# petim0/fly_bProject

Hardware: AMD Instinct MI355X
Metric: env-steps/sec (PPO rollout + update), 8192 envs per GPU (higher is better)
Workload: dtype f32 (optimizer step: fp16x2 operand split; rollout policy + critic: bf16x3 operand split; fp32 accumulate)

## Files before the change

fly_bproject_amd/_lib.py:

```python
import ctypes as C
import os

from .params import FlyParams

_HERE = os.path.dirname(os.path.abspath(__file__))
LIB_PATH = os.environ.get("FLYHIP_LIB") or os.path.join(_HERE, "libflyhip.so")
_lib = None


class FlyHipError(RuntimeError):
    pass


class FlyBuffers(C.Structure):
    _fields_ = [(n, C.c_void_p) for n in ("root", "dof_state", "targets", "contact", "pot", "prev_pot",
                                          "obs", "reward", "reset", "progress", "ep_return", "ep_length",
                                          "done_return", "done_length", "done_count")]


ABI_VERSION = 12
_P, _I, _L, _F = C.c_void_p, C.c_int, C.c_int64, C.c_float
SYMBOLS = {
    "fly_abi_version": [],
    "fly_create": [C.POINTER(FlyParams), C.POINTER(_P)],
# ... 11 lines not shown
    "ppo_step_bookkeeping": [_P, _L, _P, _F, _P, _I, _F, _F, _P],
    "ppo_rollout_step": [_P, _P, _P, _P, _P, _P, _P, _I, _F, _F, _P, _P, _P, _P, _P, _P],
    "ppo_rollout_all": [_P, _P, _P, _P, _P, _P, _P, _F, _F, _P, _P, _P, _P, _I, _P, _P, _P, _P, _P],
    "ppo_rollout_bookkeeping": [_P, _L, _L, _P, _P, _F, _P, _I, _F, _F, _P, _P],
    "mlp_forward": [_P, _P, _P, _L, _P, _P, _P, _P, _P, _P, _P, _P],
    "mlp_forward_sample": [_P, _P, _P, _L, _P, _P, _I, _F, _F, _P, _P, _P, _P, _P, _P],
    "mlp_grad_workspace_floats": [],
    "mlp_backward_dx": [_P] * 10 + [_L, _F, _F, _P, _P, _P, _P, _P, _P, _P],
    "mlp_forward_backward": [_P] * 4 + [_L] + [_P] * 9 + [_F, _F] + [_P] * 6 + [_I, _P, _P, _P, _I, _P],
    "mlp_grad_w": [_P] * 8 + [_L, _P, _P, _P, _P, _P, _P, _I, _P],
    "mlp_fused_workspace_floats": [],
    "mlp_fused_grad": [_P] * 3 + [_P, _L] + [_P] * 5 + [_F, _F] + [_P] * 6 + [C.POINTER(_P), _P],
    "mlp_fused_h2_workspace_floats": [],
    "mlp_fused_grad_h2": [_P] * 5 + [_I, _P, _L] + [_P] * 5 + [_F, _F] + [_P] * 6 + [C.POINTER(_P), _P],
    "mlp_h2_rescale": [_P] * 7,
    "mlp_adam_step": [_P] * 10 + [_F, _F, _F, _F, _F, _F, _P, _I, _P, _P, _P, _P, _P, _P] + [_P] * 3 + [_I, _P],
    "dqn_eps_greedy": [_P, _P, _P, _F, _I, _P, _L, _P],
    "dqn_huber_td": [_P, _P, _P, _P, _P, _F, _I, _L, _P, _P, _P],
    "dqn_forward": [_P, _P, _P, _L, _P, _P],
    "dqn_act": [_P, _P, _P, _L, _P, _P, _F, _P, _P, _P],
    "dqn_td_step": [_P] * 10 + [_L, _F, _F] + [_P] * 7,
    "dqn_grad_workspace_floats": [],
    "dqn_grad_w": [_P] * 6 + [_L, _P, _P, _I, _P],
    "dqn_fused_workspace_floats": [],
    "dqn_fused_image_halves": [_L],
    "dqn_fused_update": [_P] * 6 + [_I, _L, _F, _F, _P, _P, _P, _P, _I, _P],
    "dqn_fused_h2_workspace_floats": [],
    "dqn_fused_h2_image_halves": [_L],
    "dqn_fused_update_h2": [_P] * 10 + [_I, _L, _F, _F, _P, _P, _P, _P, _I, _I, _P],
    "dqn_adam_soft_update": [_P] * 12 + [_F, _F, _F, _F, _F, _P, _P, _P, _P, _P, _P, _P],
# ... 10 lines not shown
    import subprocess
    cmd = ["make", "-C", os.path.join(_HERE, "csrc"), "-j4"]
    if not verbose:
        cmd.insert(1, "-s")
    subprocess.check_call(cmd)


def load():
    global _lib
    if _lib is not None:
        return _lib
    if not os.path.exists(LIB_PATH):
        raise FlyHipError(
            "libflyhip.so is not built (%s). Run `python -c 'import __graft_entry__ as g; g.build()'` "
            "or `make -C fly_bproject_amd/csrc`. There is no CPU fallback." % LIB_PATH)
    lib = C.CDLL(LIB_PATH)
    lib.fly_last_error.restype = C.c_char_p
    lib.fly_last_error.argtypes = []
    for name, argtypes in SYMBOLS.items():
        fn = getattr(lib, name)
        fn.argtypes = argtypes
        fn.restype = C.c_int64 if name.endswith(("_workspace_floats", "_image_halves")) else C.c_int
    if lib.fly_abi_version() != ABI_VERSION:
        raise FlyHipError("stale libflyhip.so (ABI %d, this package was written for %d): rebuild it "
                          "(`make -C fly_bproject_amd/csrc`)" % (lib.fly_abi_version(), ABI_VERSION))
    _lib = lib
    return lib


def check(rc, what):
# ... 9 lines not shown
```

fly_bproject_amd/csrc/flyhip_abi.hip:

```cpp
#include <hip/hip_runtime.h>
#include <string.h>
#include <stdint.h>
#include <stdio.h>
#include <stdarg.h>
#include <new>
#include "flyhip.h"

extern "C" hipError_t flyhip_launch_env(int phases, const FlyConfig* dcfg, int n, const float* actions,
                                        const FlyBuffers* b, void* stream);
extern "C" hipError_t flyhip_launch_sample_logprob(const float* mu, const float* var, const float* eps,
                                                   float* act_out, float* logp_out, int64_t n, void* stream);
extern "C" hipError_t flyhip_launch_td_gae(const float* reward, const float* v, const float* v_next,
                                           const float* done, float gamma, float lambda, int64_t T, int64_t N,
                                           float* target_out, float* adv_out, int mode, void* stream);

extern "C" hipError_t flyhip_launch_mlp_forward(const float* P, const float* PF, const float* x, int64_t n, float* mu_out,
                                                float* v_out, float* out_save, float* h1_save, float* h2_save,
                                                float* h3_save, const uint16_t* PB, void* stream);

extern "C" hipError_t flyhip_launch_mlp_backward_dx(const float* PT, const float* out_saved, const float* h1,
                                                    const float* h2, const float* h3, const float* action,
                                                    const float* old_logp, const float* adv, const float* target,
                                                    const float* var, int64_t n, float inv_batch, float clip,
                                                    float* dz4, float* dz3, float* dz2, float* dz1, float* loss_part,
// ... 26 lines not shown
                                                   float* workspace, float* grad_out, const float* norm_mask, float* norm_ws,
                                                   int* norm_step, float* loss_part, float* const* dump, void* stream);
extern "C" hipError_t flyhip_launch_mlp_grad_w(const float* x, const float* h1, const float* h2, const float* h3,
                                               const float* dz1, const float* dz2, const float* dz3, const float* dz4,
                                               int64_t n, float* workspace, float* grad_out, const float* norm_mask,
                                               float* norm_ws, int* norm_step, const int* err, int gemm_b3, void* stream);
extern "C" hipError_t flyhip_launch_mlp_adam(float* P, float* PF, float* PT, const int* idx_f, const int* idx_t,
                                             const float* G, const float* mask, float* m,
                                             float* v, int* step, float lr, float beta1, float beta2, float eps,
                                             float max_norm, float grad_scale, float* norm_ws, int norm_ready,
                                             uint16_t* PB, uint16_t* PTB, const int* idx_fb, const int* idx_tb,
                                             int* step_out, const int* grad_invalid, uint16_t* PH, uint16_t* PTH,
                                             float* h2_scales, int h2_rescale, void* stream);
extern "C" hipError_t flyhip_launch_mlp_h2_rescale(const float* P, const int* idx_fb, const int* idx_tb, uint16_t* PH, uint16_t* PTH,
                                                   float* h2_scales, void* stream);
extern "C" int64_t flyhip_mlp_fused_h2_workspace_floats(void);
extern "C" hipError_t flyhip_launch_mlp_fused_grad_h2(const float* P, const uint16_t* PH, const uint16_t* PTH, float* fsc, int* ovf,
                                                      int freeze, const float* x, int64_t n, const float* action,
                                                      const float* old_logp, const float* adv, const float* target, const float* var,
                                                      float inv_batch, float clip, float* workspace, float* grad_out,
                                                      const float* norm_mask, float* norm_ws, int* norm_step, float* loss_part,
                                                      float* const* dump, void* stream);

extern "C" hipError_t flyhip_launch_bookkeeping(const float* reward, int64_t n, float* score_acc, float score_scale,
                                                float* action_var, int nvar, float var_decay, float var_min,
                                                void* stream);

extern "C" hipError_t flyhip_launch_dqn_eps_greedy(const float* q, const float* coin_u, const float* rand_u, float epsilon,
                                                   int A, float* act_out, int64_t n, void* stream);
extern "C" hipError_t flyhip_launch_dqn_huber_td(const float* q_table, const float* act, const float* reward,
// ... 376 lines not shown
    if (e != hipSuccess) return hip_fail(e, "mlp_fused_grad launch");
    return FLY_OK;
}

int64_t mlp_fused_h2_workspace_floats(void) { return flyhip_mlp_fused_h2_workspace_floats(); }

int mlp_h2_rescale(const float* params, const int32_t* idx_b3, const int32_t* idx_t_b3, uint16_t* params_h2, uint16_t* params_t_h2,
                   float* h2_scales, void* stream)
{
    if (!params || !idx_b3 || !idx_t_b3 || !params_h2 || !params_t_h2 || !h2_scales) return fail(FLY_E_ARG, "mlp_h2_rescale: null pointer");
    hipError_t e = flyhip_launch_mlp_h2_rescale(params, idx_b3, idx_t_b3, params_h2, params_t_h2, h2_scales, stream);
    if (e != hipSuccess) return hip_fail(e, "mlp_h2_rescale launch");
    return FLY_OK;
}

int mlp_fused_grad_h2(const float* params, const uint16_t* params_h2, const uint16_t* params_t_h2, float* h2_scales,
                      int32_t* h2_overflow, int32_t freeze, const float* x, int64_t n, const float* action,
                      const float* old_logp, const float* adv, const float* target, const float* var, float inv_batch,
                      float clip, float* workspace, float* grad, const float* norm_mask, float* norm_ws, int32_t* norm_step,
                      float* loss_part, float* const* debug_dump, void* stream)
{
    if ((norm_ws != nullptr) != (norm_mask != nullptr) || (norm_ws != nullptr) != (norm_step != nullptr))
        return fail(FLY_E_ARG, "mlp_fused_grad_h2: norm_mask, norm_ws and norm_step go together");
    if (!params || !params_h2 || !params_t_h2 || !h2_scales || !h2_overflow)
        return fail(FLY_E_ARG, "mlp_fused_grad_h2: needs params, both fp16x2 plane buffers, the scale table and the overflow word");
    if (!x || !action || !old_logp || !adv || !target || !var || !workspace || !grad)
        return fail(FLY_E_ARG, "mlp_fused_grad_h2: null pointer");
    if (n <= 0) return fail(FLY_E_ARG, "mlp_fused_grad_h2: n must be > 0");
    if (debug_dump) {
        if (!debug_dump[0]) return fail(FLY_E_ARG, "mlp_fused_grad_h2: debug_dump[0] is null");
// ... 6 lines not shown
                                                   loss_part, debug_dump, stream);
    if (e != hipSuccess) return hip_fail(e, "mlp_fused_grad_h2 launch");
    return FLY_OK;
}

int mlp_adam_step(float* params, float* params_frag, float* params_t_frag, const int32_t* idx_frag,
                  const int32_t* idx_t_frag, const float* grad, const float* mask, float* exp_avg,
                  float* exp_avg_sq, int32_t* step, float lr, float beta1, float beta2, float eps,
                  float max_norm, float grad_scale, float* norm_ws, int32_t norm_ready, uint16_t* params_b3,
                  uint16_t* params_t_b3, const int32_t* idx_b3, const int32_t* idx_t_b3, int32_t* step_out,
                  const int32_t* grad_invalid, uint16_t* params_h2, uint16_t* params_t_h2, float* h2_scales, int32_t h2_rescale,
                  void* stream)
{
    if (params_b3 && (!params_t_b3 || !idx_b3 || !idx_t_b3))
        return fail(FLY_E_ARG, "mlp_adam_step: params_b3 needs params_t_b3, idx_b3 and idx_t_b3");
    if (params_h2 && (!params_t_h2 || !h2_scales || !params_b3))
        return fail(FLY_E_ARG, "mlp_adam_step: params_h2 needs params_t_h2, h2_scales and the bf16x3 planes with their index maps");
    if (!params || !params_frag || !params_t_frag || !idx_frag || !idx_t_frag || !grad || !mask || !exp_avg ||
        !exp_avg_sq || !step || !norm_ws)
        return fail(FLY_E_ARG, "mlp_adam_step: null pointer");
    hipError_t e = flyhip_launch_mlp_adam(params, params_frag, params_t_frag, idx_frag, idx_t_frag, grad, mask, exp_avg, exp_avg_sq, step, lr, beta1, beta2,
                                          eps, max_norm, grad_scale, norm_ws, norm_ready, params_b3, params_t_b3, idx_b3, idx_t_b3,
                                          step_out, grad_invalid, params_h2, params_t_h2, h2_scales, h2_rescale, stream);
    if (e != hipSuccess) return hip_fail(e, "mlp_adam_step launch");
    return FLY_OK;
}

int dqn_eps_greedy(const float* q, const float* coin_u, const float* rand_u, float epsilon, int32_t A,
                   float* act_out, int64_t n, void* stream)
{
    if (!q || !coin_u || !rand_u || !act_out) return fail(FLY_E_ARG, "dqn_eps_greedy: null pointer");
    if (n <= 0 || A < 2) return fail(FLY_E_ARG, "dqn_eps_greedy: need n > 0 and A >= 2");
    hipError_t e = flyhip_launch_dqn_eps_greedy(q, coin_u, rand_u, epsilon, A, act_out, n, stream);
// ... 199 lines not shown
```

fly_bproject_amd/csrc/mlp_adam.inc:

```
#ifndef ADAM_THREADS_AB
#define ADAM_THREADS_AB 1024
#endif
constexpr int ADAM_THREADS = ADAM_THREADS_AB;
constexpr int ADAM_WAVES = ADAM_THREADS / 64;
constexpr int ADAM_BLOCKS = (MLP_PACKED_FLOATS + ADAM_THREADS - 1) / ADAM_THREADS;

__global__ __launch_bounds__(ADAM_THREADS) void mlp_adam_norm_kernel(const float* __restrict__ G,
                                                                     const float* __restrict__ mask, float grad_scale,
                                                                     float* __restrict__ norm_ws, int* __restrict__ step,
                                                                     const int* __restrict__ grad_invalid)
{
    __shared__ float red[ADAM_WAVES];
    if (G[MLP_ERR_SLOT] != 0.0f) return;
    if (grad_invalid && *grad_invalid != 0) return;
    const int tid = threadIdx.x;
    const int i = blockIdx.x * ADAM_THREADS + tid;
    float ss = 0.0f;
    if (i < MLP_PACKED_FLOATS) { const float g = G[i] * grad_scale * mask[i]; ss = g * g; }
    for (int o = 32; o > 0; o >>= 1) ss += __shfl_down(ss, o, 64);
    if ((tid & 63) == 0) red[tid >> 6] = ss;
    __syncthreads();
    if (tid == 0) {
        float t = 0.0f;
        for (int w = 0; w < ADAM_WAVES; ++w) t += red[w];
// ... 12 lines not shown
                                                                      const int* __restrict__ step, float lr, float beta1,
                                                                      float beta2, float eps, float max_norm,
                                                                      float grad_scale, float* __restrict__ norm_ws,
                                                                      int nparts, float part_scale,
                                                                      u16* __restrict__ PB, u16* __restrict__ PTB,
                                                                      const int* __restrict__ idx_fb,
                                                                      const int* __restrict__ idx_tb,
                                                                      int* __restrict__ step_out,
                                                                      const int* __restrict__ grad_invalid,
                                                                      u16* __restrict__ PH, u16* __restrict__ PTH,
                                                                      float* __restrict__ fsc, int h2_rescale)
{
    __shared__ float s_coef, s_step_size, s_bc2_sqrt;
    __shared__ float red[ADAM_WAVES];
    __shared__ float s_wscale[4];
    __shared__ unsigned s_wmax[4];
    const int tid = threadIdx.x;
    const bool self_norm = step_out != nullptr;
    if (G[MLP_ERR_SLOT] != 0.0f || (grad_invalid && *grad_invalid != 0)) {
        if (self_norm && blockIdx.x == 0 && tid == 0) *step_out = *step;
        return;
    }
    const int i = blockIdx.x * ADAM_THREADS + tid;
    const bool live = i < MLP_PACKED_FLOATS;
    const float mk = live ? mask[i] : 0.0f, g_in = live ? G[i] : 0.0f, m_in = live ? m[i] : 0.0f, v_in = live ? v[i] : 0.0f,
                p_in = live ? P[i] : 0.0f;
    const int jf = live ? idx_f[i] : -1, jt = live ? idx_t[i] : -1;
    {
        float t = 0.0f;
        if (self_norm) {
            const float4* g4 = reinterpret_cast<const float4*>(G);
            const float4* m4 = reinterpret_cast<const float4*>(mask);
            for (int q = tid; q < MLP_PACKED_FLOATS / 4; q += ADAM_THREADS) {
                const float4 g = g4[q], k = m4[q];
                const float a = g.x * grad_scale * k.x, b = g.y * grad_scale * k.y, c = g.z * grad_scale * k.z, d = g.w * grad_scale * k.w;
                t += (a * a + b * b) + (c * c + d * d);
            }
        } else
        for (int b = tid; b < nparts; b += ADAM_THREADS) t += norm_ws[1 + b];
        for (int o = 32; o > 0; o >>= 1) t += __shfl_down(t, o, 64);
        if ((tid & 63) == 0) red[tid >> 6] = t;
    }
    if (PH && !h2_rescale && tid < 4) s_wscale[tid] = fsc[8 + tid];
    if (PH && h2_rescale) {
        if (tid < 4) s_wmax[tid] = 0u;
        __syncthreads();
        float mx[4] = {0.0f, 0.0f, 0.0f, 0.0f};
        const float4* p4 = reinterpret_cast<const float4*>(P);
        for (int q = tid; q < MLP_PACKED_FLOATS / 4; q += ADAM_THREADS) {
            const int o = 4 * q;
            const int l = o < MLP_OFF_B1 ? 0 : o < MLP_OFF_W2 ? -1 : o < MLP_OFF_B2 ? 1 : o < MLP_OFF_W3 ? -1 : o < MLP_OFF_B3 ? 2 : o < MLP_OFF_W4 ? -1
                        : o < MLP_OFF_B4 ? 3 : -1;
            const float4 w = p4[q];
            const float a = fmaxf(fmaxf(fabsf(w.x), fabsf(w.y)), fmaxf(fabsf(w.z), fabsf(w.w)));
#pragma unroll
            for (int k = 0; k < 4; ++k) mx[k] = l == k ? fmaxf(mx[k], a) : mx[k];
        }
#pragma unroll
        for (int k = 0; k < 4; ++k) {
            float m = mx[k];
#pragma unroll
            for (int o = 32; o > 0; o >>= 1) m = fmaxf(m, __shfl_xor(m, o, 64));
            if ((tid & 63) == 0 && m > 0.0f) atomicMax(&s_wmax[k], __float_as_uint(m));
        }
        __syncthreads();
        if (tid < 4) {
            const float m = fminf(fmaxf(__uint_as_float(s_wmax[tid]), 0x1p-4f), 0x1p60f);
            const float sc = ldexpf(1.0f, 11 - ilogbf(m));
            s_wscale[tid] = sc;
            if (blockIdx.x == 0) { fsc[8 + tid] = sc; fsc[16 + 8 + tid] = 1.0f / sc; }
        }
    }
    __syncthreads();
    if (tid == 0) {
        float t = 0.0f;
        for (int w = 0; w < ADAM_WAVES; ++w) t += red[w];
        t *= part_scale;
        const float norm = sqrtf(t);
        const float coef = max_norm / (norm + 1e-6f);
        s_coef = coef < 1.0f ? coef : 1.0f;
        if (blockIdx.x == 0) norm_ws[0] = norm;
        const int step_now = self_norm ? *step + 1 : *step;
        if (self_norm && blockIdx.x == 0) *step_out = step_now;
        const float ts = (float)step_now;
        const float bc1 = 1.0f - powf(beta1, ts);
        const float bc2 = 1.0f - powf(beta2, ts);
// ... 2 lines not shown
    }
    __syncthreads();
    if (!live) return;
    const float coef = s_coef * grad_scale;
    const float step_size = s_step_size;
    const float bc2_sqrt = s_bc2_sqrt;
    const float g = g_in * coef * mk;
    const float mi = beta1 * m_in + (1.0f - beta1) * g;
    const float vi = beta2 * v_in + (1.0f - beta2) * g * g;
    m[i] = mi; v[i] = vi;
    const float denom = sqrtf(vi) / bc2_sqrt + eps;
    const float p = p_in - mk * (step_size * (mi / denom));
    P[i] = p;
    if (jf >= 0) PF[jf] = p;
    if (jt >= 0) PT[jt] = p;
    int kf = -1, kt = -1;
    if (PB) {
        u16 a, b, c;
        split3(p, a, b, c);
        kf = idx_fb[i]; kt = idx_tb[i];
        if (kf >= 0) { PB[kf] = a; PB[kf + 512] = b; PB[kf + 1024] = c; }
        if (kt >= 0) { PTB[kt] = a; PTB[kt + 512] = b; PTB[kt + 1024] = c; }
    }
    if (PH && kf >= 0) {
        const int layer = i < MLP_OFF_W2 ? 0 : i < MLP_OFF_W3 ? 1 : i < MLP_OFF_W4 ? 2 : 3;
        const float ps = p * s_wscale[layer];
        const _Float16 h0 = (_Float16)ps;
        const _Float16 h1 = (_Float16)(ps - (float)h0);
        const u16 a = __builtin_bit_cast(u16, h0), b = __builtin_bit_cast(u16, h1);
        const int hf = (kf / 1536) * 1024 + kf % 1536;
        PH[hf] = a; PH[hf + 512] = b;
        if (kt >= 0) { const int ht = (kt / 1536) * 1024 + kt % 1536; PTH[ht] = a; PTH[ht + 512] = b; }
    }
}

constexpr int H2_RESCALE_THREADS = 1024;
__global__ __launch_bounds__(H2_RESCALE_THREADS) void mlp_h2_rescale_kernel(const float* __restrict__ P, const int* __restrict__ idx_fb,
                                                                            const int* __restrict__ idx_tb, u16* __restrict__ PH,
                                                                            u16* __restrict__ PTH, float* __restrict__ fsc)
{
    __shared__ unsigned s_max[4];
    __shared__ float s_scale[4];
    const int tid = threadIdx.x;
    if (tid < 4) s_max[tid] = 0u;
    __syncthreads();
    float mine[4] = {0.0f, 0.0f, 0.0f, 0.0f};
    for (int i = tid; i < MLP_PACKED_FLOATS; i += H2_RESCALE_THREADS)
        if (idx_fb[i] >= 0) {
// ... 36 lines not shown
```

fly_bproject_amd/csrc/mlp_mfma.hip:

```cpp
#include <hip/hip_runtime.h>
#include <stdint.h>
#include <type_traits>
#include <cstdio>
#include <cstdlib>
#include "flyhip.h"
#include "mlp_layout.h"

namespace {

#include "mlp_gemm.inc"
#include "fs_stamp.inc"
#include "mlp_forward.inc"
#include "mlp_backward.inc"
#include "mlp_grad_w.inc"
#include "mlp_fused_step.inc"
#include "mlp_adam.inc"
#include "fly_body.inc"

constexpr int RS_LDS_FLOATS = FWD_LDS_FLOATS > ENVS_PER_BLOCK * FLY_NUM_OBS ? FWD_LDS_FLOATS : ENVS_PER_BLOCK * FLY_NUM_OBS;
constexpr int RS_B3_LDS_FLOATS = FWD_B3_LDS_FLOATS > ENVS_PER_BLOCK * FLY_NUM_OBS ? FWD_B3_LDS_FLOATS : ENVS_PER_BLOCK * FLY_NUM_OBS;
static_assert(ENVS_PER_BLOCK == BM && BLOCK == THREADS, "one forward tile = one env block");

template <bool B3>
__global__ __launch_bounds__(THREADS, B3 ? 1 : 2) void rollout_step_kernel(
// ... 450 lines not shown
                                             float* h2_scales, int h2_rescale, void* stream)
{
    int nparts = ADAM_BLOCKS;
    float part_scale = 1.0f;
    if (step_out) {
        part_scale = 1.0f;
    } else if (norm_ready) {
        nparts = RED_BLOCKS;
        part_scale = grad_scale * grad_scale;
    } else {
        hipLaunchKernelGGL(mlp_adam_norm_kernel, dim3(ADAM_BLOCKS), dim3(ADAM_THREADS), 0, (hipStream_t)stream, G, mask,
                           grad_scale, norm_ws, step, grad_invalid);
        hipError_t e = hipGetLastError();
        if (e != hipSuccess) return e;
    }
    hipLaunchKernelGGL(mlp_adam_apply_kernel, dim3(ADAM_BLOCKS), dim3(ADAM_THREADS), 0, (hipStream_t)stream, P, PF, PT,
                       idx_f, idx_t, G, mask, m, v, step, lr, beta1, beta2, eps, max_norm, grad_scale, norm_ws, nparts,
                       part_scale, PB, PTB, idx_fb, idx_tb, step_out, grad_invalid, PH, PTH, h2_scales, h2_rescale);
    return hipGetLastError();
}

extern "C" hipError_t flyhip_launch_mlp_h2_rescale(const float* P, const int* idx_fb, const int* idx_tb, uint16_t* PH, uint16_t* PTH,
                                                   float* h2_scales, void* stream)
{
    hipLaunchKernelGGL(mlp_h2_rescale_kernel, dim3(1), dim3(H2_RESCALE_THREADS), 0, (hipStream_t)stream, P, idx_fb, idx_tb, PH, PTH, h2_scales);
    return hipGetLastError();
}
```

fly_bproject_amd/policy.py:

```python
import ctypes as C
import os

import torch

from . import _lib

IN, IN_PAD, H1, H2, H3, OUT, NACT = 73, 80, 256, 128, 128, 32, 18
OFF_W1 = 0
OFF_B1 = OFF_W1 + H1 * IN_PAD
OFF_W2 = OFF_B1 + H1
OFF_B2 = OFF_W2 + H2 * H1
OFF_W3 = OFF_B2 + H2
OFF_B3 = OFF_W3 + H3 * H2
OFF_W4 = OFF_B3 + H3
OFF_B4 = OFF_W4 + OUT * H3
PACKED = OFF_B4 + OUT
ERR_SLOT = OFF_W1 + 76
OFF_F1 = 0
OFF_F2 = OFF_F1 + H1 * IN_PAD
OFF_F3 = OFF_F2 + H2 * H1
OFF_F4 = OFF_F3 + H3 * H2
FRAG = OFF_F4 + OUT * H3
OFF_TF2 = 0
OFF_TF3 = OFF_TF2 + H1 * H2
# ... 50 lines not shown
        src = off_w + n * K + k
        if li == 1:
            idx_fb[src] = OFF_PB[li] + (k // 128) * (3 * N * 128) + _plane_index(n, k % 128, 128)
        else:
            idx_fb[src] = OFF_PB[li] + _plane_index(n, k, K)
        if OFF_PTB[li] is not None:
            idx_tb[src] = OFF_PTB[li] + _plane_index(k, n, N)
    for idx, size in ((idx_fb, PB_HALVES), (idx_tb, PTB_HALVES)):
        used = idx[idx >= 0].astype(np.int64)
        allpos = np.concatenate([used, used + 512, used + 1024])
        assert len(np.unique(allpos)) == len(allpos) and allpos.max() < size
    assert 3 * (idx_fb >= 0).sum() == PB_HALVES and 3 * (idx_tb >= 0).sum() == PTB_HALVES
    return idx_fb, idx_tb


PH_HALVES, PTH_HALVES = PB_HALVES * 2 // 3, PTB_HALVES * 2 // 3
H2_SCALE_FLOATS, H2_INV, H2_W0 = 48, 16, 8
H2_CLASSES = ("x", "h1", "h2", "h3", "dz4", "dz3", "dz2", "dz1")


def split_f16x2(w, scale):
    y = w * scale
    h0 = y.to(torch.float16)
    h1 = (y - h0.float()).to(torch.float16)
    return [t.view(torch.int16) for t in (h0, h1)]


def h2_weight_scale(wmax):
    import math
    m = min(max(float(wmax), 2.0 ** -4), 2.0 ** 60)
# ... 9 lines not shown


def split_bf16x3(w):
    w0 = w.to(torch.bfloat16)
    r1 = w - w0.float()
    w1 = r1.to(torch.bfloat16)
    w2 = (r1 - w1.float()).to(torch.bfloat16)
    return [t.view(torch.int16) for t in (w0, w1, w2)]


class PackedPolicy:
    def __init__(self, net, device):
        self.device = torch.device(device)
        self._lib = _lib.load()
        self.P = torch.zeros(PACKED, dtype=torch.float32, device=self.device)
        self.PF = torch.zeros(FRAG, dtype=torch.float32, device=self.device)
        self.PT = torch.zeros(FRAG_T, dtype=torch.float32, device=self.device)
        env_gemm = os.environ.get("FLY_GEMM")
        self._gemm = "bf16x3" if env_gemm in (None, "f16x2") else env_gemm
        self.gemm_infer = os.environ.get("FLY_GEMM_INFER", self._gemm)
        assert self._gemm in ("f32", "bf16x3") and self.gemm_infer in ("f32", "bf16x3")
        self.PB = torch.zeros(PB_HALVES, dtype=torch.int16, device=self.device)
        self.PTB = torch.zeros(PTB_HALVES, dtype=torch.int16, device=self.device)
        self._step_gemm = os.environ.get("FLY_STEP_GEMM", "f16x2" if env_gemm in (None, "f16x2") else "bf16x3")
        assert self._step_gemm in ("bf16x3", "f16x2")
        self.PH = torch.zeros(PH_HALVES, dtype=torch.int16, device=self.device)
        self.PTH = torch.zeros(PTH_HALVES, dtype=torch.int16, device=self.device)
        self.h2_scales = torch.zeros(H2_SCALE_FLOATS, dtype=torch.float32, device=self.device)
        self.h2_overflow = torch.zeros(1, dtype=torch.int32, device=self.device)
        self.h2_freeze = False
        self.h2_calibrated = False
        self._h2_steps_since_rescale = 0
        self.h2_suspended = False
        self.h2_overflows = 0
        self._h2_reset_scales()
        idx_fb, idx_tb = build_plane_maps()
        self.idx_fb = torch.from_numpy(idx_fb).to(self.device)
        self.idx_tb = torch.from_numpy(idx_tb).to(self.device)
        self._src_fb = torch.nonzero(self.idx_fb >= 0).squeeze(-1)
        self._dst_fb = self.idx_fb[self._src_fb].long()
        self._src_tb = torch.nonzero(self.idx_tb >= 0).squeeze(-1)
        self._dst_tb = self.idx_tb[self._src_tb].long()
        idx_f, idx_t = build_index_maps()
        self.idx_f = torch.from_numpy(idx_f).to(self.device)
        self.idx_t = torch.from_numpy(idx_t).to(self.device)
        self._src_f = torch.nonzero(self.idx_f >= 0).squeeze(-1)
        self._dst_f = self.idx_f[self._src_f].long()
        self._src_t = torch.nonzero(self.idx_t >= 0).squeeze(-1)
        self._dst_t = self.idx_t[self._src_t].long()
        P = self.P
        self.W1 = P[OFF_W1:OFF_B1].view(H1, IN_PAD)
        self.b1 = P[OFF_B1:OFF_W2]
        self.W2 = P[OFF_W2:OFF_B2].view(H2, H1)
        self.b2 = P[OFF_B2:OFF_W3]
        self.W3 = P[OFF_W3:OFF_B3].view(H3, H2)
        self.b3 = P[OFF_B3:OFF_W4]
        self.W4 = P[OFF_W4:OFF_B4].view(OUT, H3)
        self.b4 = P[OFF_B4:PACKED]
        self.views = {
            "shared_net.0.weight": self.W1[:, :IN], "shared_net.0.bias": self.b1,
            "shared_net.2.weight": self.W2, "shared_net.2.bias": self.b2,
            "to_mean.0.weight": self.W3[:64], "to_mean.0.bias": self.b3[:64],
            "to_value.0.weight": self.W3[64:], "to_value.0.bias": self.b3[64:],
            "to_mean.2.weight": self.W4[:NACT, :64], "to_mean.2.bias": self.b4[:NACT],
# ... 2 lines not shown
        params = dict(net.named_parameters())
        assert set(params) == set(self.views), "Net does not have the reference's parameter set"
        with torch.no_grad():
            for k, view in self.views.items():
                view.copy_(params[k].data.to(self.device))
                params[k].data = view
        mask = torch.zeros(PACKED, dtype=torch.float32, device=self.device)
        for k, view in self.views.items():
            off = view.storage_offset()
            idx = torch.arange(PACKED, device=self.device).as_strided(view.shape, view.stride(), off)
            mask[idx.reshape(-1)] = 1.0
        self.grad_mask = mask
        assert int(mask.sum().item()) == 69587
        self.refresh()

    def refresh(self):
        with torch.no_grad():
            self.PF[self._dst_f] = self.P[self._src_f]
            self.PT[self._dst_t] = self.P[self._src_t]
            self._refresh_planes()
        self.version += 1

    refresh_transposes = refresh

    def _refresh_planes(self):
        with torch.no_grad():
            for dst_buf, src, dst in ((self.PB, self._src_fb, self._dst_fb), (self.PTB, self._src_tb, self._dst_tb)):
                for term, plane in enumerate(split_bf16x3(self.P[src])):
                    dst_buf[dst + 512 * term] = plane

        if self.h2_live():
# ... 6 lines not shown
        s = torch.ones(H2_SCALE_FLOATS)
        s[:4] = 2.0 ** 4
        s[4:8] = 2.0 ** 28
        s[H2_INV:H2_INV + 16] = 1.0 / s[:16]
        s[32:] = 0.0
        self.h2_scales.copy_(s)
        self.h2_calibrated = False

    def _refresh_planes_h2(self):
        if self.device.type != "cuda":
            return
        p = lambda t: C.c_void_p(t.data_ptr())
        _lib.check(self._lib.mlp_h2_rescale(p(self.P), p(self.idx_fb), p(self.idx_tb), p(self.PH), p(self.PTH), p(self.h2_scales),
                                            _lib.stream_ptr()), "mlp_h2_rescale")
        self._h2_steps_since_rescale = 0

    def _planes_live(self):
        return self._gemm == "bf16x3" or self.gemm_infer == "bf16x3"

    @property
    def step_gemm(self):
        return self._step_gemm if self._gemm == "bf16x3" else self._gemm

    @step_gemm.setter
    def step_gemm(self, mode):
        assert mode in ("bf16x3", "f16x2")
        was = self.h2_live()
        self._step_gemm = mode
        if self.h2_live() and not was:
            self._refresh_planes_h2()
# ... 18 lines not shown
        elif self.h2_live() and not was_h2:
            self._refresh_planes_h2()
    version = 0

    def _plane_args(self):
        if not self._planes_live():
            return (None, None, None, None)
        p = lambda t: C.c_void_p(t.data_ptr())
        return (p(self.PB), p(self.PTB), p(self.idx_fb), p(self.idx_tb))

    def _h2_args(self):
        if not self.h2_live():
            return (None, None, None, C.c_int(0))
        p = lambda t: C.c_void_p(t.data_ptr())
        rescale = self._h2_steps_since_rescale >= max(1, min(64, int(0.9 / (3.2 * self.lr))))
        self._h2_steps_since_rescale = 1 if rescale else self._h2_steps_since_rescale + 1
        return (p(self.PH), p(self.PTH), p(self.h2_scales), C.c_int(1 if rescale else 0))

    def pb_ptr(self):
        return C.c_void_p(self.PB.data_ptr()) if self.gemm == "bf16x3" else None

    def infer_pb_ptr(self):
        return C.c_void_p(self.PB.data_ptr()) if self.gemm_infer == "bf16x3" else None

    def ptb_ptr(self):
        return C.c_void_p(self.PTB.data_ptr()) if self.gemm == "bf16x3" else None

    def forward(self, x, want_mu=True, want_v=True, saves=None):
        lead = x.shape[:-1]
        x2 = x.reshape(-1, IN)
# ... 155 lines not shown
        return (parts[0] + parts[1]) / n

    @property
    def step(self):
        return self._step2[self._step_idx:self._step_idx + 1]

    def adam_step(self, grad_scale=1.0, norm_ready=False, self_norm=False, grad_invalid=None):
        p = lambda t: C.c_void_p(t.data_ptr())
        self.version += 1
        self.steps_issued += 1
        step_in = self.step
        step_out = None
        if self_norm:
            self._step_idx ^= 1
            step_out = p(self.step)
        _lib.check(self._lib.mlp_adam_step(p(self.P), p(self.PF), p(self.PT), p(self.idx_f), p(self.idx_t), p(self.G),
                                           p(self.grad_mask), p(self.exp_avg),
                                           p(self.exp_avg_sq), p(step_in), C.c_float(self.lr),
                                           C.c_float(self.betas[0]), C.c_float(self.betas[1]), C.c_float(self.eps),
                                           C.c_float(self.max_norm), C.c_float(grad_scale), p(self._norm_ws),
                                           C.c_int(1 if norm_ready else 0), *self._plane_args(), step_out,
                                           p(grad_invalid) if grad_invalid is not None else None, *self._h2_args(), _lib.stream_ptr()),
                   "mlp_adam_step")
```

fly_bproject_amd/ppo.py:

```python
import ctypes as C
import collections
import os

import torch
import torch.nn as nn
import torch.nn.functional as F

from . import _lib
from .fly import Fly
from .params import NUM_DOF


class Net(nn.Module):

    def __init__(self, num_obs, num_act):
        super().__init__()
        self.shared_net = nn.Sequential(nn.Linear(num_obs, 256), nn.ELU(), nn.Linear(256, 128), nn.ELU())
        self.to_mean = nn.Sequential(nn.Linear(128, 64), nn.ELU(), nn.Linear(64, num_act), nn.ELU())
        self.to_value = nn.Sequential(nn.Linear(128, 64), nn.ELU(), nn.Linear(64, 1))

    _policy = None

    def pi(self, x):
        if self._policy is not None and not torch.is_grad_enabled():
# ... 279 lines not shown
                pol.check_fused_launch()
            if short == 0:
                break
            if short < 0 or short > len(slices) or attempt == 2:
                raise _lib.FlyHipError("update: device step counter is %d steps behind the %d issued" % (short, pol.steps_issued))
            pol.steps_issued -= short
            if h2 and not pol.h2_suspended:
                pol.h2_overflow.zero_()
                pol.h2_suspended = True
                pol.h2_calibrated = False
                pol.h2_overflows += 1
            else:
                pol.fuse_fwd_bwd = False
                print("mlp_forward_backward: %d of %d optimizer steps were refused on the device (a backward workgroup "
                      "could not get its tile); redoing them with two launches" % (short, len(slices)))
            run(slices[len(slices) - short:])
            if self._p2p is not None and not self._p2p.check():
                raise _lib.FlyHipError("dp_allreduce_p2p: a rank never published its gradient while refused steps were redone")
        pol.h2_suspended = False
        self.optim_step += len(slices)
        self._drain_log(block=True)
        self._finish_update(sync_grads)

    def _finish_update(self, sync_grads):
        import torch.distributed as dist
        pol = self.policy
        if self.world_size > 1 and not sync_grads:
            for buf in (pol.P, pol.exp_avg, pol.exp_avg_sq):
                dist.all_reduce(buf, op=dist.ReduceOp.SUM)
                buf.div_(self.world_size)
            pol.refresh()

    def prepare(self):
        if getattr(self, "_prepared", False):
            return
        self._prepared = True
        self.p2p_selftest = None
        sync_grads = self.world_size > 1 and self.dp_mode == "grad_allreduce"
        if sync_grads and self.update_backend == "hip" and self.dp_allreduce in ("p2p", "auto"):
            self._p2p = self._open_p2p(self.policy.G.numel())

# ... 257 lines not shown
```

include/flyhip.h:

```cpp
#ifndef FLYHIP_H
#define FLYHIP_H

#include <stdint.h>

#ifdef __cplusplus
extern "C" {
#endif

#define FLY_NUM_DOF 18
#define FLY_NUM_OBS 73
#define FLY_NUM_LEGS 6
#define FLY_NUM_ABDOMEN 5
#define FLY_NUM_CONTACT 11
#define FLY_ROOT_DIM 13

#define FLY_OK 0
#define FLY_E_ARG (-1)
#define FLY_E_HIP (-2)
#define FLY_E_CONFIG (-3)

#define PPO_GAE_COMPAT 0
#define PPO_GAE_DONE_PER_STEP 1
#define PPO_GAE_MASK_RECURRENCE 2
#define PPO_GAE_SCAN 4
// ... 134 lines not shown
                   float inv_batch, float clip, float* workspace, float* grad, const float* norm_mask, float* norm_ws,
                   int32_t* norm_step, float* loss_part, float* const* debug_dump, void* stream);
int mlp_adam_step(float* params, float* params_frag, float* params_t_frag, const int32_t* idx_frag,
                  const int32_t* idx_t_frag, const float* grad, const float* mask, float* exp_avg,
                  float* exp_avg_sq, int32_t* step, float lr, float beta1, float beta2, float eps,
                  float max_norm, float grad_scale, float* norm_ws, int32_t norm_ready,
                  uint16_t* params_b3, uint16_t* params_t_b3, const int32_t* idx_b3,
                  const int32_t* idx_t_b3, int32_t* step_out, const int32_t* grad_invalid,
                  uint16_t* params_h2, uint16_t* params_t_h2, float* h2_scales, int32_t h2_rescale, void* stream);

#define MLP_PH_HALVES_ABI 147456
#define MLP_PTH_HALVES_ABI 106496
#define MLP_H2_SCALE_FLOATS_ABI 48
int mlp_h2_rescale(const float* params, const int32_t* idx_b3, const int32_t* idx_t_b3, uint16_t* params_h2, uint16_t* params_t_h2,
                   float* h2_scales, void* stream);
int64_t mlp_fused_h2_workspace_floats(void);
int mlp_fused_grad_h2(const float* params, const uint16_t* params_h2, const uint16_t* params_t_h2, float* h2_scales,
                      int32_t* h2_overflow, int32_t freeze, const float* x, int64_t n, const float* action,
                      const float* old_logp, const float* adv, const float* target, const float* var, float inv_batch,
                      float clip, float* workspace, float* grad, const float* norm_mask, float* norm_ws, int32_t* norm_step,
                      float* loss_part, float* const* debug_dump, void* stream);


int dqn_eps_greedy(const float* q, const float* coin_u, const float* rand_u, float epsilon, int32_t A,
                   float* act_out, int64_t n, void* stream);
int dqn_huber_td(const float* q_table, const float* act, const float* reward, const float* q_next,
                 const float* done, float discount, int32_t A, int64_t B, float* dq, float* loss_part,
                 void* stream);

#define DQN_QB_HALVES_ABI 282624
// ... 51 lines not shown
```

Before: 68.06 million.

## Defer fp32/bf16x3 plane writes out of Adam into a lazy refresh kernel

```diff
diff --git a/fly_bproject_amd/_lib.py b/fly_bproject_amd/_lib.py
--- a/fly_bproject_amd/_lib.py
+++ b/fly_bproject_amd/_lib.py
@@ -49,6 +49,7 @@
     "mlp_fused_h2_workspace_floats": [],
     "mlp_fused_grad_h2": [_P] * 5 + [_I, _P, _L] + [_P] * 5 + [_F, _F] + [_P] * 6 + [C.POINTER(_P), _P],
     "mlp_h2_rescale": [_P] * 7,
+    "mlp_plane_refresh": [_P] * 7,
     "mlp_adam_step": [_P] * 10 + [_F, _F, _F, _F, _F, _F, _P, _I, _P, _P, _P, _P, _P, _P] + [_P] * 3 + [_I, _P],
     "dqn_eps_greedy": [_P, _P, _P, _F, _I, _P, _L, _P],
     "dqn_huber_td": [_P, _P, _P, _P, _P, _F, _I, _L, _P, _P, _P],
@@ -89,6 +90,7 @@
         raise FlyHipError(
             "libflyhip.so is not built (%s). Run `python -c 'import __graft_entry__ as g; g.build()'` "
             "or `make -C fly_bproject_amd/csrc`. There is no CPU fallback." % LIB_PATH)
+    import torch
     lib = C.CDLL(LIB_PATH)
     lib.fly_last_error.restype = C.c_char_p
     lib.fly_last_error.argtypes = []
diff --git a/fly_bproject_amd/csrc/flyhip_abi.hip b/fly_bproject_amd/csrc/flyhip_abi.hip
--- a/fly_bproject_amd/csrc/flyhip_abi.hip
+++ b/fly_bproject_amd/csrc/flyhip_abi.hip
@@ -64,6 +64,8 @@
                                              float* h2_scales, int h2_rescale, void* stream);
 extern "C" hipError_t flyhip_launch_mlp_h2_rescale(const float* P, const int* idx_fb, const int* idx_tb, uint16_t* PH, uint16_t* PTH,
                                                    float* h2_scales, void* stream);
+extern "C" hipError_t flyhip_launch_mlp_plane_refresh(const float* P, const int* src, float* PF, float* PT, uint16_t* PB, uint16_t* PTB,
+                                                     void* stream);
 extern "C" int64_t flyhip_mlp_fused_h2_workspace_floats(void);
 extern "C" hipError_t flyhip_launch_mlp_fused_grad_h2(const float* P, const uint16_t* PH, const uint16_t* PTH, float* fsc, int* ovf,
                                                       int freeze, const float* x, int64_t n, const float* action,
@@ -470,6 +472,16 @@
     return FLY_OK;
 }
 
+int mlp_plane_refresh(const float* params, const int32_t* src_map, float* params_frag, float* params_t_frag, uint16_t* params_b3,
+                      uint16_t* params_t_b3, void* stream)
+{
+    if (!params || !src_map || !params_frag || !params_t_frag || !params_b3 || !params_t_b3)
+        return fail(FLY_E_ARG, "mlp_plane_refresh: null pointer");
+    hipError_t e = flyhip_launch_mlp_plane_refresh(params, src_map, params_frag, params_t_frag, params_b3, params_t_b3, stream);
+    if (e != hipSuccess) return hip_fail(e, "mlp_plane_refresh launch");
+    return FLY_OK;
+}
+
 int mlp_fused_grad_h2(const float* params, const uint16_t* params_h2, const uint16_t* params_t_h2, float* h2_scales,
                       int32_t* h2_overflow, int32_t freeze, const float* x, int64_t n, const float* action,
                       const float* old_logp, const float* adv, const float* target, const float* var, float inv_batch,
@@ -506,9 +518,10 @@
 {
     if (params_b3 && (!params_t_b3 || !idx_b3 || !idx_t_b3))
         return fail(FLY_E_ARG, "mlp_adam_step: params_b3 needs params_t_b3, idx_b3 and idx_t_b3");
-    if (params_h2 && (!params_t_h2 || !h2_scales || !params_b3))
-        return fail(FLY_E_ARG, "mlp_adam_step: params_h2 needs params_t_h2, h2_scales and the bf16x3 planes with their index maps");
-    if (!params || !params_frag || !params_t_frag || !idx_frag || !idx_t_frag || !grad || !mask || !exp_avg ||
+    if (params_h2 && (!params_t_h2 || !h2_scales || !idx_b3 || !idx_t_b3))
+        return fail(FLY_E_ARG, "mlp_adam_step: params_h2 needs params_t_h2, h2_scales and the bf16x3 index maps");
+    const bool lean = params_h2 && !params_frag && !params_t_frag && !params_b3 && !params_t_b3;
+    if (!params || (!lean && (!params_frag || !params_t_frag)) || !idx_frag || !idx_t_frag || !grad || !mask || !exp_avg ||
         !exp_avg_sq || !step || !norm_ws)
         return fail(FLY_E_ARG, "mlp_adam_step: null pointer");
     hipError_t e = flyhip_launch_mlp_adam(params, params_frag, params_t_frag, idx_frag, idx_t_frag, grad, mask, exp_avg, exp_avg_sq, step, lr, beta1, beta2,
diff --git a/fly_bproject_amd/csrc/mlp_adam.inc b/fly_bproject_amd/csrc/mlp_adam.inc
--- a/fly_bproject_amd/csrc/mlp_adam.inc
+++ b/fly_bproject_amd/csrc/mlp_adam.inc
@@ -3,6 +3,7 @@
 #endif
 constexpr int ADAM_THREADS = ADAM_THREADS_AB;
 constexpr int ADAM_WAVES = ADAM_THREADS / 64;
+constexpr int H2_WMAX_SLOT = 40;
 constexpr int ADAM_BLOCKS = (MLP_PACKED_FLOATS + ADAM_THREADS - 1) / ADAM_THREADS;
 
 __global__ __launch_bounds__(ADAM_THREADS) void mlp_adam_norm_kernel(const float* __restrict__ G,
@@ -50,7 +51,6 @@
     __shared__ float s_coef, s_step_size, s_bc2_sqrt;
     __shared__ float red[ADAM_WAVES];
     __shared__ float s_wscale[4];
-    __shared__ unsigned s_wmax[4];
     const int tid = threadIdx.x;
     const bool self_norm = step_out != nullptr;
     if (G[MLP_ERR_SLOT] != 0.0f || (grad_invalid && *grad_invalid != 0)) {
@@ -61,7 +61,8 @@
     const bool live = i < MLP_PACKED_FLOATS;
     const float mk = live ? mask[i] : 0.0f, g_in = live ? G[i] : 0.0f, m_in = live ? m[i] : 0.0f, v_in = live ? v[i] : 0.0f,
                 p_in = live ? P[i] : 0.0f;
-    const int jf = live ? idx_f[i] : -1, jt = live ? idx_t[i] : -1;
+    const int jf = live && PF ? idx_f[i] : -1, jt = live && PF ? idx_t[i] : -1;
+    const int kf = live && (PB || PH) ? idx_fb[i] : -1, kt = live && (PB || PH) ? idx_tb[i] : -1;
     {
         float t = 0.0f;
         if (self_norm) {
@@ -77,35 +78,14 @@
         for (int o = 32; o > 0; o >>= 1) t += __shfl_down(t, o, 64);
         if ((tid & 63) == 0) red[tid >> 6] = t;
     }
-    if (PH && !h2_rescale && tid < 4) s_wscale[tid] = fsc[8 + tid];
-    if (PH && h2_rescale) {
-        if (tid < 4) s_wmax[tid] = 0u;
-        __syncthreads();
-        float mx[4] = {0.0f, 0.0f, 0.0f, 0.0f};
-        const float4* p4 = reinterpret_cast<const float4*>(P);
-        for (int q = tid; q < MLP_PACKED_FLOATS / 4; q += ADAM_THREADS) {
-            const int o = 4 * q;
-            const int l = o < MLP_OFF_B1 ? 0 : o < MLP_OFF_W2 ? -1 : o < MLP_OFF_B2 ? 1 : o < MLP_OFF_W3 ? -1 : o < MLP_OFF_B3 ? 2 : o < MLP_OFF_W4 ? -1
-                        : o < MLP_OFF_B4 ? 3 : -1;
-            const float4 w = p4[q];
-            const float a = fmaxf(fmaxf(fabsf(w.x), fabsf(w.y)), fmaxf(fabsf(w.z), fabsf(w.w)));
-#pragma unroll
-            for (int k = 0; k < 4; ++k) mx[k] = l == k ? fmaxf(mx[k], a) : mx[k];
-        }
-#pragma unroll
-        for (int k = 0; k < 4; ++k) {
-            float m = mx[k];
-#pragma unroll
-            for (int o = 32; o > 0; o >>= 1) m = fmaxf(m, __shfl_xor(m, o, 64));
-            if ((tid & 63) == 0 && m > 0.0f) atomicMax(&s_wmax[k], __float_as_uint(m));
-        }
-        __syncthreads();
-        if (tid < 4) {
-            const float m = fminf(fmaxf(__uint_as_float(s_wmax[tid]), 0x1p-4f), 0x1p60f);
-            const float sc = ldexpf(1.0f, 11 - ilogbf(m));
-            s_wscale[tid] = sc;
+    if (PH && tid < 4) {
+        float sc = fsc[8 + tid];
+        if (h2_rescale) {
+            const float m = fminf(fmaxf(fsc[H2_WMAX_SLOT + tid], 0x1p-4f), 0x1p60f);
+            sc = ldexpf(1.0f, 11 - ilogbf(m));
             if (blockIdx.x == 0) { fsc[8 + tid] = sc; fsc[16 + 8 + tid] = 1.0f / sc; }
         }
+        s_wscale[tid] = sc;
     }
     __syncthreads();
     if (tid == 0) {
@@ -138,11 +118,9 @@
     P[i] = p;
     if (jf >= 0) PF[jf] = p;
     if (jt >= 0) PT[jt] = p;
-    int kf = -1, kt = -1;
     if (PB) {
         u16 a, b, c;
         split3(p, a, b, c);
-        kf = idx_fb[i]; kt = idx_tb[i];
         if (kf >= 0) { PB[kf] = a; PB[kf + 512] = b; PB[kf + 1024] = c; }
         if (kt >= 0) { PTB[kt] = a; PTB[kt + 512] = b; PTB[kt + 1024] = c; }
     }
@@ -156,6 +134,60 @@
         PH[hf] = a; PH[hf + 512] = b;
         if (kt >= 0) { const int ht = (kt / 1536) * 1024 + kt % 1536; PTH[ht] = a; PTH[ht + 512] = b; }
     }
+}
+
+constexpr int H2_WMAX_THREADS = 1024;
+__global__ __launch_bounds__(H2_WMAX_THREADS) void mlp_h2_wmax_kernel(const float* __restrict__ P, float* __restrict__ fsc)
+{
+    __shared__ unsigned s_wmax[4];
+    const int tid = threadIdx.x;
+    if (tid < 4) s_wmax[tid] = 0u;
+    __syncthreads();
+    float mx[4] = {0.0f, 0.0f, 0.0f, 0.0f};
+    const float4* p4 = reinterpret_cast<const float4*>(P);
+    for (int q = tid; q < MLP_PACKED_FLOATS / 4; q += H2_WMAX_THREADS) {
+        const int o = 4 * q;
+        const int l = o < MLP_OFF_B1 ? 0 : o < MLP_OFF_W2 ? -1 : o < MLP_OFF_B2 ? 1 : o < MLP_OFF_W3 ? -1 : o < MLP_OFF_B3 ? 2 : o < MLP_OFF_W4 ? -1
+                    : o < MLP_OFF_B4 ? 3 : -1;
+        const float4 w = p4[q];
+        const float a = fmaxf(fmaxf(fabsf(w.x), fabsf(w.y)), fmaxf(fabsf(w.z), fabsf(w.w)));
+#pragma unroll
+        for (int k = 0; k < 4; ++k) mx[k] = l == k ? fmaxf(mx[k], a) : mx[k];
+    }
+#pragma unroll
+    for (int k = 0; k < 4; ++k) {
+        float m = mx[k];
+#pragma unroll
+        for (int o = 32; o > 0; o >>= 1) m = fmaxf(m, __shfl_xor(m, o, 64));
+        if ((tid & 63) == 0 && m > 0.0f) atomicMax(&s_wmax[k], __float_as_uint(m));
+    }
+    __syncthreads();
+    if (tid < 4) fsc[H2_WMAX_SLOT + tid] = __uint_as_float(s_wmax[tid]);
+}
+
+constexpr int PLANE_REFRESH_THREADS = 256;
+constexpr int MLP_PLANE_REFRESH_ITEMS = MLP_FRAG_FLOATS + MLP_FRAG_T_FLOATS + MLP_PB_HALVES / 3 + MLP_PTB_HALVES / 3;
+static_assert(MLP_PB_HALVES % 1536 == 0 && MLP_PTB_HALVES % 1536 == 0 && MLP_FRAG_FLOATS % 64 == 0 && MLP_FRAG_T_FLOATS % 64 == 0,
+              "whole 1536-word blocks, wave-aligned segments");
+__global__ __launch_bounds__(PLANE_REFRESH_THREADS) void mlp_plane_refresh_kernel(const float* __restrict__ P, const int* __restrict__ src,
+                                                                                  float* __restrict__ PF, float* __restrict__ PT,
+                                                                                  u16* __restrict__ PB, u16* __restrict__ PTB)
+{
+    const int d = blockIdx.x * PLANE_REFRESH_THREADS + threadIdx.x;
+    if (d >= MLP_PLANE_REFRESH_ITEMS) return;
+    const int j = src[d];
+    if (j < 0) return;
+    const float p = P[j];
+    if (d < MLP_FRAG_FLOATS) { PF[d] = p; return; }
+    int e = d - MLP_FRAG_FLOATS;
+    if (e < MLP_FRAG_T_FLOATS) { PT[e] = p; return; }
+    e -= MLP_FRAG_T_FLOATS;
+    u16* dst = PB;
+    if (e >= MLP_PB_HALVES / 3) { e -= MLP_PB_HALVES / 3; dst = PTB; }
+    u16 a, b, c;
+    split3(p, a, b, c);
+    u16* w = dst + (e / 512) * 1536 + e % 512;
+    w[0] = a; w[512] = b; w[1024] = c;
 }
 
 constexpr int H2_RESCALE_THREADS = 1024;
diff --git a/fly_bproject_amd/csrc/mlp_mfma.hip b/fly_bproject_amd/csrc/mlp_mfma.hip
--- a/fly_bproject_amd/csrc/mlp_mfma.hip
+++ b/fly_bproject_amd/csrc/mlp_mfma.hip
@@ -488,12 +488,26 @@
         hipError_t e = hipGetLastError();
         if (e != hipSuccess) return e;
     }
+    if (PH && h2_rescale) {
+        hipLaunchKernelGGL(mlp_h2_wmax_kernel, dim3(1), dim3(H2_WMAX_THREADS), 0, (hipStream_t)stream, P, h2_scales);
+        hipError_t e = hipGetLastError();
+        if (e != hipSuccess) return e;
+    }
     hipLaunchKernelGGL(mlp_adam_apply_kernel, dim3(ADAM_BLOCKS), dim3(ADAM_THREADS), 0, (hipStream_t)stream, P, PF, PT,
                        idx_f, idx_t, G, mask, m, v, step, lr, beta1, beta2, eps, max_norm, grad_scale, norm_ws, nparts,
                        part_scale, PB, PTB, idx_fb, idx_tb, step_out, grad_invalid, PH, PTH, h2_scales, h2_rescale);
     return hipGetLastError();
 }
 
+static_assert(MLP_PLANE_REFRESH_ITEMS == MLP_PLANE_REFRESH_ITEMS_ABI, "include/flyhip.h states the refresh map's length");
+extern "C" hipError_t flyhip_launch_mlp_plane_refresh(const float* P, const int* src, float* PF, float* PT, uint16_t* PB, uint16_t* PTB,
+                                                     void* stream)
+{
+    hipLaunchKernelGGL(mlp_plane_refresh_kernel, dim3((MLP_PLANE_REFRESH_ITEMS + PLANE_REFRESH_THREADS - 1) / PLANE_REFRESH_THREADS),
+                       dim3(PLANE_REFRESH_THREADS), 0, (hipStream_t)stream, P, src, PF, PT, PB, PTB);
+    return hipGetLastError();
+}
+
 extern "C" hipError_t flyhip_launch_mlp_h2_rescale(const float* P, const int* idx_fb, const int* idx_tb, uint16_t* PH, uint16_t* PTH,
                                                    float* h2_scales, void* stream)
 {
diff --git a/fly_bproject_amd/policy.py b/fly_bproject_amd/policy.py
--- a/fly_bproject_amd/policy.py
+++ b/fly_bproject_amd/policy.py
@@ -88,6 +88,20 @@
     return idx_fb, idx_tb
 
 
+def build_refresh_map(idx_f, idx_t, idx_fb, idx_tb):
+    import numpy as np
+    parts = []
+    for idx, size, planes in ((idx_f, FRAG, False), (idx_t, FRAG_T, False), (idx_fb, PB_HALVES // 3, True), (idx_tb, PTB_HALVES // 3, True)):
+        inv = np.full(size, -1, np.int32)
+        src = np.nonzero(idx >= 0)[0]
+        dst = idx[src].astype(np.int64)
+        if planes:
+            dst = (dst // 1536) * 512 + dst % 1536
+        inv[dst] = src
+        parts.append(inv)
+    return np.concatenate(parts)
+
+
 PH_HALVES, PTH_HALVES = PB_HALVES * 2 // 3, PTB_HALVES * 2 // 3
 H2_SCALE_FLOATS, H2_INV, H2_W0 = 48, 16, 8
 H2_CLASSES = ("x", "h1", "h2", "h3", "dz4", "dz3", "dz2", "dz1")
@@ -127,14 +141,16 @@
         self.device = torch.device(device)
         self._lib = _lib.load()
         self.P = torch.zeros(PACKED, dtype=torch.float32, device=self.device)
-        self.PF = torch.zeros(FRAG, dtype=torch.float32, device=self.device)
-        self.PT = torch.zeros(FRAG_T, dtype=torch.float32, device=self.device)
+        self._planes_stale = False
+        self.lean_adam = os.environ.get("FLY_LEAN_ADAM", "1") != "0"
+        self._PF = torch.zeros(FRAG, dtype=torch.float32, device=self.device)
+        self._PT = torch.zeros(FRAG_T, dtype=torch.float32, device=self.device)
         env_gemm = os.environ.get("FLY_GEMM")
         self._gemm = "bf16x3" if env_gemm in (None, "f16x2") else env_gemm
         self.gemm_infer = os.environ.get("FLY_GEMM_INFER", self._gemm)
         assert self._gemm in ("f32", "bf16x3") and self.gemm_infer in ("f32", "bf16x3")
-        self.PB = torch.zeros(PB_HALVES, dtype=torch.int16, device=self.device)
-        self.PTB = torch.zeros(PTB_HALVES, dtype=torch.int16, device=self.device)
+        self._PB = torch.zeros(PB_HALVES, dtype=torch.int16, device=self.device)
+        self._PTB = torch.zeros(PTB_HALVES, dtype=torch.int16, device=self.device)
         self._step_gemm = os.environ.get("FLY_STEP_GEMM", "f16x2" if env_gemm in (None, "f16x2") else "bf16x3")
         assert self._step_gemm in ("bf16x3", "f16x2")
         self.PH = torch.zeros(PH_HALVES, dtype=torch.int16, device=self.device)
@@ -144,6 +160,7 @@
         self.h2_freeze = False
         self.h2_calibrated = False
         self._h2_steps_since_rescale = 0
+        self._h2_rescale_issued = None
         self.h2_suspended = False
         self.h2_overflows = 0
         self._h2_reset_scales()
@@ -161,6 +178,7 @@
         self._dst_f = self.idx_f[self._src_f].long()
         self._src_t = torch.nonzero(self.idx_t >= 0).squeeze(-1)
         self._dst_t = self.idx_t[self._src_t].long()
+        self._refresh_src = torch.from_numpy(build_refresh_map(idx_f, idx_t, idx_fb, idx_tb)).to(self.device)
         P = self.P
         self.W1 = P[OFF_W1:OFF_B1].view(H1, IN_PAD)
         self.b1 = P[OFF_B1:OFF_W2]
@@ -193,7 +211,36 @@
         assert int(mask.sum().item()) == 69587
         self.refresh()
 
+    @property
+    def PF(self):
+        self.sync_planes()
+        return self._PF
+
+    @property
+    def PT(self):
+        self.sync_planes()
+        return self._PT
+
+    @property
+    def PB(self):
+        self.sync_planes()
+        return self._PB
+
+    @property
+    def PTB(self):
+        self.sync_planes()
+        return self._PTB
+
+    def sync_planes(self):
+        if not self._planes_stale:
+            return
+        self._planes_stale = False
+        p = lambda t: C.c_void_p(t.data_ptr())
+        _lib.check(self._lib.mlp_plane_refresh(p(self.P), p(self._refresh_src), p(self._PF), p(self._PT), p(self._PB), p(self._PTB),
+                                               _lib.stream_ptr()), "mlp_plane_refresh")
+
     def refresh(self):
+        self._planes_stale = False
         with torch.no_grad():
             self.PF[self._dst_f] = self.P[self._src_f]
             self.PT[self._dst_t] = self.P[self._src_t]
@@ -230,6 +277,7 @@
         _lib.check(self._lib.mlp_h2_rescale(p(self.P), p(self.idx_fb), p(self.idx_tb), p(self.PH), p(self.PTH), p(self.h2_scales),
                                             _lib.stream_ptr()), "mlp_h2_rescale")
         self._h2_steps_since_rescale = 0
+        self._h2_rescale_issued = None
 
     def _planes_live(self):
         return self._gemm == "bf16x3" or self.gemm_infer == "bf16x3"
@@ -278,6 +326,10 @@
             return (None, None, None, C.c_int(0))
         p = lambda t: C.c_void_p(t.data_ptr())
         rescale = self._h2_steps_since_rescale >= max(1, min(64, int(0.9 / (3.2 * self.lr))))
+        if self._h2_rescale_issued is not None and self._h2_rescale_issued >= self.steps_issued:
+            rescale = True
+        if rescale:
+            self._h2_rescale_issued = self.steps_issued
         self._h2_steps_since_rescale = 1 if rescale else self._h2_steps_since_rescale + 1
         return (p(self.PH), p(self.PTH), p(self.h2_scales), C.c_int(1 if rescale else 0))
 
@@ -463,11 +515,19 @@
         if self_norm:
             self._step_idx ^= 1
             step_out = p(self.step)
-        _lib.check(self._lib.mlp_adam_step(p(self.P), p(self.PF), p(self.PT), p(self.idx_f), p(self.idx_t), p(self.G),
+        lean = self.lean_adam and self.fused_step and self.h2_live() and not self.h2_suspended
+        if lean:
+            frag, planes = (None, None), (None, None, p(self.idx_fb), p(self.idx_tb))
+        else:
+            frag, planes = (p(self.PF), p(self.PT)), self._plane_args()
+        h2 = self._h2_args()
+        _lib.check(self._lib.mlp_adam_step(p(self.P), *frag, p(self.idx_f), p(self.idx_t), p(self.G),
                                            p(self.grad_mask), p(self.exp_avg),
                                            p(self.exp_avg_sq), p(step_in), C.c_float(self.lr),
                                            C.c_float(self.betas[0]), C.c_float(self.betas[1]), C.c_float(self.eps),
                                            C.c_float(self.max_norm), C.c_float(grad_scale), p(self._norm_ws),
-                                           C.c_int(1 if norm_ready else 0), *self._plane_args(), step_out,
-                                           p(grad_invalid) if grad_invalid is not None else None, *self._h2_args(), _lib.stream_ptr()),
+                                           C.c_int(1 if norm_ready else 0), *planes, step_out,
+                                           p(grad_invalid) if grad_invalid is not None else None, *h2, _lib.stream_ptr()),
                    "mlp_adam_step")
+        if lean:
+            self._planes_stale = True
diff --git a/fly_bproject_amd/ppo.py b/fly_bproject_amd/ppo.py
--- a/fly_bproject_amd/ppo.py
+++ b/fly_bproject_amd/ppo.py
@@ -317,6 +317,7 @@
                 pol.fuse_fwd_bwd = False
                 print("mlp_forward_backward: %d of %d optimizer steps were refused on the device (a backward workgroup "
                       "could not get its tile); redoing them with two launches" % (short, len(slices)))
+            pol.sync_planes()
             run(slices[len(slices) - short:])
             if self._p2p is not None and not self._p2p.check():
                 raise _lib.FlyHipError("dp_allreduce_p2p: a rank never published its gradient while refused steps were redone")
@@ -328,6 +329,7 @@
     def _finish_update(self, sync_grads):
         import torch.distributed as dist
         pol = self.policy
+        pol.sync_planes()
         if self.world_size > 1 and not sync_grads:
             for buf in (pol.P, pol.exp_avg, pol.exp_avg_sq):
                 dist.all_reduce(buf, op=dist.ReduceOp.SUM)
diff --git a/include/flyhip.h b/include/flyhip.h
--- a/include/flyhip.h
+++ b/include/flyhip.h
@@ -172,6 +172,9 @@
 #define MLP_H2_SCALE_FLOATS_ABI 48
 int mlp_h2_rescale(const float* params, const int32_t* idx_b3, const int32_t* idx_t_b3, uint16_t* params_h2, uint16_t* params_t_h2,
                    float* h2_scales, void* stream);
+#define MLP_PLANE_REFRESH_ITEMS_ABI 253952
+int mlp_plane_refresh(const float* params, const int32_t* src_map, float* params_frag, float* params_t_frag, uint16_t* params_b3,
+                      uint16_t* params_t_b3, void* stream);
 int64_t mlp_fused_h2_workspace_floats(void);
 int mlp_fused_grad_h2(const float* params, const uint16_t* params_h2, const uint16_t* params_t_h2, float* h2_scales,
                       int32_t* h2_overflow, int32_t freeze, const float* x, int64_t n, const float* action,
```

New measurement: 68.68 million, median of 6. No clear change (+0.9%).
